# hooman007/ProtoASNet

Measured on AMD Instinct MI355X. Metric: clips/sec forward, higher is better.
Workload: dtype bf16; 1 GPU; Video ProtoASNet forward, x3d_s trunk + prototype layer (P=30, D=256, K=3), 32x16x224x224 echo clips per GPU; global_batch=32, parallelism=dp1 (independent clips, no collective), launch=hipGraph replay of the forward's launch list (one graph launch per step)

## Files before the change

protoasnet_amd/csrc/stem_mfma.hip:

```cpp
#include "common.h"
#include "igemm_epilogue.h"

namespace pasn {

constexpr int SM_ROWS = 4, SM_COLS = 56, SM_PC = 116, SM_PR = 2 * (SM_ROWS - 1) + 3, SM_RING = 6;
static_assert(SM_PC % 4 == 0 && SM_PC >= 2 * SM_COLS + 4, "whole 4-column staging units, every window inside the patch");
constexpr int SM_PF = 3;

template <typename TIN>
struct SmRaw;
template <>
struct SmRaw<float> {
    f32x4 v;
    __device__ void load(const float* p) { v = *reinterpret_cast<const f32x4*>(p); }
    __device__ float get(int e) const { return v[e]; }
};
template <>
struct SmRaw<__bf16> {
    bf16x4 v;
    __device__ void load(const __bf16* p) { v = *reinterpret_cast<const bf16x4*>(p); }
    __device__ float get(int e) const { return (float)v[e]; }
};
template <>
struct SmRaw<unsigned char> {
    unsigned v;
    __device__ void load(const unsigned char* p) { v = *reinterpret_cast<const unsigned*>(p); }
    __device__ float get(int e) const { return (float)((v >> (8 * e)) & 0xffu); }
};

template <typename TIN, int CIN>
__global__ __launch_bounds__(256, 2) void x3d_stem_mfma_kernel(const TIN* __restrict__ x, const __bf16* __restrict__ wq,
                                                               const float* __restrict__ scale, const float* __restrict__ bias,
                                                               __bf16* __restrict__ y, pasn_conv_desc d, float in_a, float in_b) {
    constexpr int NT = 1, MT = 2, BN = 32, OROW = BN + 8;
    constexpr int RPF = CIN * 3;
    constexpr int KROWS = 5 * RPF;
    constexpr int KS = (KROWS + 3) / 4;
    constexpr int SLOT = CIN * SM_PR * SM_PC;
    constexpr int UNITS = SLOT / 4;
    constexpr int UPT = (UNITS + 255) / 256;
    extern __shared__ __attribute__((aligned(16))) char smem[];
    __bf16* const ring = reinterpret_cast<__bf16*>(smem);
    __bf16* const imgs = reinterpret_cast<__bf16*>(smem + SM_RING * SLOT * 2);
    float* const scb = reinterpret_cast<float*>(smem + SM_RING * SLOT * 2 + 4 * 32 * OROW * 2);
    const int tid = threadIdx.x, lane = tid & 63, wave = __builtin_amdgcn_readfirstlane(tid >> 6);
    const int c = lane & 31, h = lane >> 5;
    const int T = d.Ti;

    const int ncol = (d.Wo + SM_COLS - 1) / SM_COLS, nrow = (d.Ho + SM_ROWS - 1) / SM_ROWS;
    int b = blockIdx.x;
    const int ct = b % ncol;
    b /= ncol;
    const int rt = b % nrow;
    const int n = b / nrow;
    const int oh0 = rt * SM_ROWS, ow0 = ct * SM_COLS;
    const int hi_base = oh0 * 2 - 1, wi_base = ow0 * 2 - 4;

    bf16x8 wa[KS];
#pragma unroll
    for (int s = 0; s < KS; ++s) wa[s] = *reinterpret_cast<const bf16x8*>(wq + ((size_t)(2 * s + h) * BN + c) * 8);
    igemm_stage_scale_bias<BN>(scb, scale, bias, 0, d.Cout_p, tid);

    const long plane = (long)d.Hi * d.Wi;
    int uoff[UPT];
    int uci[UPT];
#pragma unroll
    for (int k = 0; k < UPT; ++k) {
        const int u = tid + 256 * k;
        const int pc4 = u % (SM_PC / 4), r = (u / (SM_PC / 4)) % SM_PR, ci = u / ((SM_PC / 4) * SM_PR);
        const int hi = hi_base + r, wi = wi_base + pc4 * 4;
        const bool ok = u < UNITS && (unsigned)hi < (unsigned)d.Hi && (unsigned)wi < (unsigned)d.Wi;
        uoff[k] = ok ? hi * d.Wi + wi : -1;
        uci[k] = ci < CIN ? ci : CIN - 1;
    }
    SmRaw<TIN> raw[UPT];
    auto fetch = [&](int ti) {
#pragma unroll
        for (int k = 0; k < UPT; ++k)
            raw[k].load(x + (((long)n * CIN + uci[k]) * T + ti) * plane + (uoff[k] >= 0 ? uoff[k] : 0));
    };
    auto stage = [&](int slot, bool inside) {
        __bf16* dst = ring + slot * SLOT;
#pragma unroll
        for (int k = 0; k < UPT; ++k) {
            const int u = tid + 256 * k;
            float v[4];
#pragma unroll
            for (int e = 0; e < 4; ++e) v[e] = (inside && uoff[k] >= 0) ? fmaf(raw[k].get(e), in_a, in_b) : 0.0f;
            if (u < UNITS) store4(dst + u * 4, v);
        }
    };

    const int lane_off = (2 * wave) * SM_PC + 2 * c + 2;
    const int oh = oh0 + wave;
    const int cgs = d.Cout_p / 8;
    __bf16* const img = imgs + (size_t)wave * 32 * OROW;

    auto emit = [&](int to, const int (&sb)[5]) {
        f32x16 acc[NT][MT];
#pragma unroll
        for (int j = 0; j < MT; ++j)
#pragma unroll
            for (int r = 0; r < 16; ++r) acc[0][j][r] = 0.0f;
#pragma unroll
        for (int s = 0; s < KS; ++s) {
            auto rowoff = [&](int R) {
                const int Rc = R < KROWS ? R : KROWS - 1;
                return sb[Rc / RPF] + (((Rc % RPF) / 3) * SM_PR + (Rc % RPF) % 3) * SM_PC;
            };
            const int oa = h ? rowoff(4 * s + 2) : rowoff(4 * s + 0);
            const int ob = h ? rowoff(4 * s + 3) : rowoff(4 * s + 1);
            const __bf16* srca = ring + lane_off + oa;
            const __bf16* srcb = ring + lane_off + ob;
            bf16x8 bfr[MT];
#pragma unroll
            for (int j = 0; j < MT; ++j) {
                typedef unsigned u32x4 __attribute__((ext_vector_type(4)));
                const unsigned* pa = reinterpret_cast<const unsigned*>(srca + 64 * j);
                const unsigned* pb = reinterpret_cast<const unsigned*>(srcb + 64 * j);
                u32x4 v;
                v.x = pa[0];
                v.y = pa[1];
                v.z = pb[0];
                v.w = pb[1];
                bfr[j] = __builtin_bit_cast(bf16x8, v);
            }
#pragma unroll
            for (int j = 0; j < MT; ++j) mma32(acc[0][j], wa[s], bfr[j]);
        }
        __builtin_amdgcn_sched_group_barrier(0x100, 2 * MT * SM_PF, 0);
#pragma unroll
        for (int s = 0; s < KS; ++s) {
            __builtin_amdgcn_sched_group_barrier(0x008, MT, 0);
            if (s + SM_PF < KS) __builtin_amdgcn_sched_group_barrier(0x100, 2 * MT, 0);
        }
        igemm_epilogue<NT, MT>(acc, img, scb, nullptr, y, 0, cgs, d, lane, [&](int j, long& mbase, int& nvalid) {
            mbase = (((long)n * d.To + to) * d.Ho + oh) * d.Wo + ow0 + 32 * j;
            nvalid = oh < d.Ho ? min(min(32, SM_COLS - 32 * j), d.Wo - (ow0 + 32 * j)) : 0;
        });
    };

    const int nf = T + 4;
    int r = 0;
#pragma unroll 1
    for (int f = 0; f < nf; ++f) {
        const int ti = f - 2;
        stage(r, ti >= 0 && ti < T);
        if (ti + 1 >= 0 && ti + 1 < T) fetch(ti + 1);
        __syncthreads();
        const int to = f - 4;
        if (to >= 0) {
            int sb[5];
#pragma unroll
            for (int kt = 0; kt < 5; ++kt) {
                int q = r + 2 + kt;
                q = q >= SM_RING ? q - SM_RING : q;
                q = q >= SM_RING ? q - SM_RING : q;
                sb[kt] = q * SLOT;
            }
            emit(to, sb);
        }
        r = r + 1 == SM_RING ? 0 : r + 1;
    }
}

int x3d_stem_mfma_supported(const pasn_conv_desc& d, int out_dtype) {
    if (const char* e = tune("PASN_NO_STEM_MFMA"))
        if (e[0] == '1') return 0;
    if (out_dtype != PASN_BF16 || (d.Cin != 1 && d.Cin != 3) || d.Cout_p > 32) return 0;
    if (d.kt != 1 || d.kh != 3 || d.kw != 3 || d.st != 1 || d.sh != 2 || d.sw != 2 || d.pt != 0 || d.ph != 1 || d.pw != 1) return 0;
    if (d.Wi % 4 != 0 || d.To != d.Ti) return 0;
    if ((long)d.N * d.Cin * d.Ti * d.Hi * d.Wi >= (1L << 31)) return 0;
    return 1;
}

template <typename TIN>
static int launch_stem_mfma_t(const void* x, const void* wq, const float* scale, const float* bias, void* y, const pasn_conv_desc& d,
                              float in_a, float in_b, hipStream_t s) {
    const size_t slot = (size_t)d.Cin * SM_PR * SM_PC * 2;
    const size_t lds = SM_RING * slot + (size_t)4 * 32 * (32 + 8) * 2 + 32 * 8;
    const dim3 grid((unsigned)((long)d.N * ceil_div(d.Ho, SM_ROWS) * ceil_div(d.Wo, SM_COLS))), block(256);
    if (d.Cin == 3) {
        PASN_MAX_LDS(96 * 1024, x3d_stem_mfma_kernel<TIN, 3>);
        hipLaunchKernelGGL((x3d_stem_mfma_kernel<TIN, 3>), grid, block, lds, s, (const TIN*)x, (const __bf16*)wq, scale, bias, (__bf16*)y, d,
                           in_a, in_b);
    } else {
        hipLaunchKernelGGL((x3d_stem_mfma_kernel<TIN, 1>), grid, block, lds, s, (const TIN*)x, (const __bf16*)wq, scale, bias, (__bf16*)y, d,
                           in_a, in_b);
    }
    return check_launch("x3d_stem_mfma_kernel");
}

int launch_x3d_stem_mfma(const void* x, const void* wq, const float* scale, const float* bias, void* y, const pasn_conv_desc& d, int in_dtype,
                         float in_a, float in_b, hipStream_t s) {
    if (in_dtype == PASN_F32) return launch_stem_mfma_t<float>(x, wq, scale, bias, y, d, in_a, in_b, s);
    if (in_dtype == PASN_BF16) return launch_stem_mfma_t<__bf16>(x, wq, scale, bias, y, d, in_a, in_b, s);
    if (in_dtype == PASN_U8) return launch_stem_mfma_t<unsigned char>(x, wq, scale, bias, y, d, in_a, in_b, s);
    set_error("x3d_stem_mfma: unknown input dtype");
    return PASN_ERR_ARG;
}

}
```

protoasnet_amd/csrc/tuning.hip:

```cpp
#include "tuning.h"

#include <stdlib.h>
#include <string.h>

#include <map>
#include <mutex>
#include <string>

#include "common.h"

extern char** environ;

namespace pasn {

struct TuneEntry {
    const char* name;
    const char* cls;
    const char* doc;
};

static const TuneEntry kRegistry[] = {
    {"PASN_DWMFMA",           "route", "0: depthwise 3x3x3 stride-1 stencil on the VALU kernels instead of the matrix-core kernel (dwmfma.hip)"},
    {"PASN_DWMFMA_MAXW",      "route", "matrix-core stencil only on planes at most this wide"},
    {"PASN_DW_STATS_MFMA",    "route", "0: training forward takes the stencil's batch statistics on the VALU kernel"},
    {"PASN_DW_DGRAD_REDUCE",  "route", "0: depthwise dgrad without the fused backward sums of the producer unit"},
    {"PASN_DWWG_FUSED",       "route", "1: depthwise weight gradient with the three kt taps in one launch"},
    {"PASN_EXPDW",            "route", "0: no fused expand-conv + stencil launch (x3d_expdw.hip)"},
    {"PASN_DW_TEMPORAL",      "route", "0: depthwise (kt,1,1) convs on the generic strip kernel instead of the T-marching kernel (dwtemporal.hip)"},
    {"PASN_DW_TZ",            "route", "0: the stride-1 stencils of planes 9 .. 14 wide on dwconv3d_mfma_kernel instead of the Toeplitz kernel (dw_tz.hip); 1: the Toeplitz kernel also where its blocks do not fit one round (more than 512)"},
    {"PASN_EXPDW_TZ",         "route", "0: stride-1 fused expand + stencil launches on the block-diagonal kernel (x3d_expdw.hip) instead of the Toeplitz kernel (x3d_expdw_tz.hip)"},
    {"PASN_EXPDW_S1",         "route", "stride-1 use of the fused expand + stencil launch: 0 off, 1 the SE blocks of wide planes only"},
    {"PASN_EXPDW_FUSE",       "route", "0: fused expand + stencil step as two scheduling regions (expand, then stencil)"},
    {"PASN_EXPDW_FOLD",       "route", "0: norm_a's scale applied in the fused launch's epilogue instead of folded into the expand weights (host side, plan.py)"},
    {"PASN_HEAD_CHAIN",       "route", "0: head B as seven launches instead of the chained launch (head_chain.hip)"},
    {"PASN_NO_DGRAD_S2",      "route", "stride-2 depthwise dgrad through the generic kernel"},
    {"PASN_NO_DWMARCH",       "route", "no T-marching VALU stencil (dwmarch.hip)"},
    {"PASN_NO_DWWG_MARCH",    "route", "depthwise weight gradient without the T-marching kernel"},
    {"PASN_NO_DWWG_STRIP",    "route", "depthwise weight gradient without the strip kernel"},
    {"PASN_NO_DW_STATS",      "route", "training forward: stencil and batch statistics as two calls"},
    {"PASN_NO_FC_MFMA",       "route", "7x7 stems on the VALU kernel instead of first_conv_mfma.hip"},
    {"PASN_NO_FIRST_IM2COL",  "route", "first-layer weight gradient without the im2col path"},
    {"PASN_NO_GEMM",          "route", "no LDS-tiled GEMM for pointwise convs (gemm_pw.hip)"},
    {"PASN_NO_GEMM_BN64",     "route", "no 64-column instance of the LDS-tiled GEMM"},
    {"PASN_TCONV",            "route", "0: temporal (3,1,1) convs on the implicit-GEMM kernels instead of the weight-stationary T-marching kernel (tconv_ws.hip)"},
    {"PASN_NO_HALO",          "route", "no halo-tile implicit GEMM (igemm_halo.hip)"},
    {"PASN_NO_IGEMM",         "route", "no direct-to-LDS implicit GEMM (igemm.hip)"},
    {"PASN_NO_PACK",          "route", "1: training weights packed by torch ops instead of the one-launch pack kernel (host side, train.py)"},
    {"PASN_WGT_WIDE",         "geom",  "0: the wide pointwise weight gradient with one 32 x 32 tile per wave everywhere (no 1 x 2 / 2 x 1 tiles per wave along the wide side)"},
    {"PASN_WGT_XCD",          "geom",  "0: the wide pointwise weight gradient's tile groups as blockIdx.y (a sweep apart) instead of back to back on one XCD"},
    {"PASN_DWWG_MARCH2",      "route", "0: depthwise weight gradient by round 2's marching kernel instead of round 4's (dw_wgrad.hip)"},
    {"PASN_DWWG_CH",          "geom",  "channels per thread of the depthwise weight-gradient march (4 default, 2)"},
    {"PASN_DWWG_WT",          "geom",  "outputs per strip of the depthwise weight-gradient march at stride 1 (2 default, 3)"},
    {"PASN_DWWG_BLOCKS",      "geom",  "cap on the blocks (= partial rows) of the depthwise weight-gradient march (default 512)"},
    {"PASN_TRAIN_BLOCKS",     "geom",  "blocks an elementwise training pass is cut into (default 1024; the partial-sum workspaces scale with it)"},
    {"PASN_TRAIN_ROWS_CONTIG", "geom", "1: the elementwise training passes map Cp / 8 lanes to a row (contiguous spans, fewer idle lanes) instead of the next power of two"},
    {"PASN_NO_TRAIN_PAIR",    "route", "1: the loss recipe's two trunk passes of a training step as two passes instead of one paired pass with two statistics groups (host side, trainer.py)"},
    {"PASN_TRAIN_STREAMS",    "route", "1: weight-gradient launches of the training step on the main stream instead of a second one (host side, train.py)"},
    {"PASN_TRAIN_SIDE_DEPTH", "geom",  "side-stream weight-gradient launches outstanding before the main stream waits (default 2)"},
    {"PASN_NO_EDP",           "route", "1: no whole-block launch for the 7 x 7 stage (x3d_edp.hip)"},
    {"PASN_NO_PE",            "route", "1: no streamed project + expand pair launch for the 432-channel stage (x3d_pe.hip)"},
    {"PASN_NO_PWCONV",        "route", "no register-resident persistent pointwise conv (pwconv.hip)"},
    {"PASN_NO_PWTINY",        "route", "no one-wave-per-tile pointwise conv for small maps (pwconv_tiny.hip)"},
    {"PASN_NO_SE_ANALYTIC",   "route", "training: squeeze-excite backward without the analytic pooled-gradient path (host side, train.py)"},
    {"PASN_NO_SE_FUSE",       "route", "squeeze-excite gate never inside the stencil launch"},
    {"PASN_NO_SE_PROLOGUE",   "route", "squeeze-excite gate never in the project conv's prologue"},
    {"PASN_NO_SHORTFUSE",     "route", "strided shortcut conv as its own launch"},
    {"PASN_NO_STEM",          "route", "X3D stem as two launches"},
    {"PASN_NO_STEM_MFMA",     "route", "X3D stem on the VALU kernel instead of stem_mfma.hip"},
    {"PASN_NO_TAIL_MFMA",     "route", "training head tail without the matrix-core pooling"},
    {"PASN_NO_WGRAD_GATHER",  "route", "windowed weight gradient without the gather kernel"},
    {"PASN_NO_WGRAD_HALO",    "route", "windowed weight gradient without the halo kernel (wgrad_halo.hip)"},
    {"PASN_NO_WGRAD_LDS",     "route", "pointwise weight gradient without the LDS kernel"},
    {"PASN_NO_WGRAD_TILE",    "route", "windowed weight gradient without the tiled kernel"},
    {"PASN_NO_XPAIR",         "route", "project conv never chained with the next expand conv (pwconv_xpair.hip)"},
    {"PASN_NO_XTILE",         "route", "no X-stationary pointwise conv (pwconv_xtile.hip)"},
    {"PASN_POOL_VALU",        "route", "1: head-B pooling on the VALU kernel"},
    {"PASN_SE_FUSE_MAXC",     "route", "largest channel count whose squeeze-excite gate rides in the stencil launch (default 128)"},
    {"PASN_WGRAD_DET",        "route", "1: windowed weight gradient through fixed-order partial buffers only"},
    {"PASN_WS",               "route", "0: no weight-stationary pointwise conv (pwconv_ws.hip); 'all': every covered layer"},
    {"PASN_WSPAIR",           "route", "0: no chained pairs in the weight-stationary kernel"},
    {"PASN_WS_GATED",         "route", "0: gated (SE / Swish input) layers not on the weight-stationary kernel"},
    {"PASN_XPAIR_ALL",        "route", "1: chain every covered project / expand pair, also the narrow stage-3 ones"},
    {"PASN_XTILE_GATED",      "route", "0: gated layers not on the X-stationary kernel"},
    {"PASN_DWMFMA_TC",        "geom",  "matrix-core stencil: forced T chunk"},
    {"PASN_DWMFMA_UPB",       "geom",  "matrix-core stencil: forced units per block"},
    {"PASN_DWM_TC",           "geom",  "VALU marching stencil: forced T chunk"},
    {"PASN_DWM_WT",           "geom",  "VALU marching stencil: forced outputs per strip"},
    {"PASN_EXPDW_TC",         "geom",  "fused expand + stencil: forced T chunk"},
    {"PASN_EXPDW_UPB",        "geom",  "fused expand + stencil: forced units per block"},
    {"PASN_WS_BPC",           "geom",  "weight-stationary conv: forced blocks per channel group"},
    {"PASN_WS_MT",            "geom",  "weight-stationary conv: forced 32-row sub-tiles per wave"},
    {"PASN_WS_NS",            "geom",  "weight-stationary conv: forced stage count"},
    {"PASN_WS_PT",            "geom",  "weight-stationary conv: forced waves along positions"},
    {"PASN_WS_MINK",          "geom",  "weight-stationary conv: smallest padded K it takes (default 48)"},
    {"PASN_PE_MT",            "geom",  "streamed project + expand pair: 32-row tiles per unit (2 or 4, default 4)"},
    {"PASN_DWMFMA_ABL",       "dev",   "matrix-core stencil timing ablations (bit mask)"},
    {"PASN_EXPDW_ABL",        "dev",   "fused expand + stencil timing ablations (bit mask)"},
    {"PASN_HALO_ABL",         "dev",   "halo implicit GEMM timing ablations"},
    {"PASN_PW_ABL",           "dev",   "persistent pointwise conv timing ablations (bit mask)"},
    {"PASN_WS_ABL",           "dev",   "weight-stationary conv timing ablations (needs -DPASN_WS_ABLATE too)"},
    {"PASN_EDP_STAMPS",       "dev",   "whole-block launch of the 7 x 7 stage: in-kernel phase stamps (tools/edp_bench.py)"},
    {"PASN_TZ_STAMPS",        "dev",   "Toeplitz expand + stencil launch: in-kernel phase stamps (tools/tz_bench.py)"},
    {"PASN_PE_STAMPS",        "dev",   "streamed project + expand pair: in-kernel phase stamps (tools/pe_bench.py)"},
    {"PASN_DW_WT",            "dev",   "strip stencil: outputs per thread (4, 7, 8)"},
    {"PASN_HALO_SP",          "dev",   "halo implicit GEMM: slice pipeline on / off"},
    {"PASN_IGEMM_NT",         "dev",   "implicit GEMM: forced channel tiles per block"},
    {"PASN_IGEMM_RR",         "dev",   "implicit GEMM: round-robin tile order"},
    {"PASN_WGT_BLOCKS",       "dev",   "tiled weight gradient: target block count"},
    {"PASN_WG_TPW",           "dev",   "tiled weight gradient: tiles per wave cap"},
    {"PASN_WS_HELP",          "dev",   "weight-stationary conv: 0 = no helper waves for the input transform"},
    {"PASN_WS_ROWS",          "dev",   "weight-stationary conv: minimum rows per block"},
    {"PASN_XT_MINK",          "dev",   "X-stationary conv: smallest padded K it takes"},
};

struct Snapshot {
    std::map<std::string, std::string> set;
    std::string unknown;
};

static std::mutex g_mu;
static Snapshot* g_snap = nullptr;

static bool host_side_name(const char* n) {
    static const char* const kHost[] = {"PASN_LIB_PATH", "PASN_EXTRA_HIPCC_FLAGS", "PASN_NATIVE_RCCL", "PASN_BENCH_BACKEND", "PASN_PARITY_LOG", "PASN_TB_TORCHPROF", "PASN_KB_ACT", "PASN_HC_ABL"};
    for (const char* h : kHost)
        if (!strcmp(h, n)) return true;
    return false;
}

static Snapshot* take_snapshot() {
    Snapshot* s = new Snapshot;
    for (char** e = environ; e && *e; ++e) {
        if (strncmp(*e, "PASN_", 5)) continue;
        const char* eq = strchr(*e, '=');
        if (!eq) continue;
        const std::string name(*e, eq - *e);
        bool known = false;
        for (const TuneEntry& t : kRegistry)
            if (name == t.name) {
                known = true;
#ifndef PASN_TUNING
                if (!strcmp(t.cls, "dev")) break;
#endif
                s->set[name] = eq + 1;
                break;
            }
        if (!known && !host_side_name(name.c_str())) s->unknown += (s->unknown.empty() ? "" : " ") + name;
    }
    return s;
}

static Snapshot* snapshot() {
    std::lock_guard<std::mutex> lk(g_mu);
    if (!g_snap) g_snap = take_snapshot();
    return g_snap;
}

const char* tune(const char* name) {
    Snapshot* s = snapshot();
    if (s->set.empty()) return nullptr;
    const auto it = s->set.find(name);
    return it == s->set.end() ? nullptr : it->second.c_str();
}

}

using namespace pasn;

extern "C" void pasn_tuning_reload(void) {
    Snapshot* s = take_snapshot();
    std::lock_guard<std::mutex> lk(g_mu);
    g_snap = s;
}

extern "C" const char* pasn_tuning_get(const char* name) { return name ? tune(name) : nullptr; }

extern "C" int pasn_tuning_report(char* buf, int cap, int with_registry) {
    Snapshot* s = snapshot();
    std::string out;
    for (const auto& kv : s->set) out += kv.first + "=" + kv.second + "\n";
    if (!s->unknown.empty()) out += "unknown: " + s->unknown + "\n";
    if (with_registry)
        for (const TuneEntry& t : kRegistry) out += std::string(t.name) + "\t" + t.cls + "\t" + t.doc + "\n";
    if (buf && cap > 0) {
        const int n = (int)out.size() < cap - 1 ? (int)out.size() : cap - 1;
        memcpy(buf, out.data(), n);
        buf[n] = 0;
    }
    return (int)out.size();
}
```

Before: 12750 clips/s.

## Restructure X3D stem frame pipeline with prologue lead fetch and stage-after-MFMA

Reworks the stem's temporal loop. A prologue fetches and stages the first three frames up front, and the steady-state loop then runs the MFMA K-loop before staging the next frame into the ring, so global loads and LDS stores overlap the matrix work instead of preceding it. Per-unit offsets become advancing pointers plus an in-bounds bitmask, which cuts address arithmetic. Also adds dev-only ablation flags, compiled out unless PASN_TUNING is defined, at the cost of more registers held by the lead buffers in the prologue.

```diff
diff --git a/protoasnet_amd/csrc/stem_mfma.hip b/protoasnet_amd/csrc/stem_mfma.hip
--- a/protoasnet_amd/csrc/stem_mfma.hip
+++ b/protoasnet_amd/csrc/stem_mfma.hip
@@ -6,6 +6,15 @@
 constexpr int SM_ROWS = 4, SM_COLS = 56, SM_PC = 116, SM_PR = 2 * (SM_ROWS - 1) + 3, SM_RING = 6;
 static_assert(SM_PC % 4 == 0 && SM_PC >= 2 * SM_COLS + 4, "whole 4-column staging units, every window inside the patch");
 constexpr int SM_PF = 3;
+constexpr int SM_LEAD = 3;
+
+#ifdef PASN_TUNING
+#define PASN_STEM_ABL_PARAM , int abl
+#define PASN_STEM_ABL_VALUE , stem_abl
+#else
+#define PASN_STEM_ABL_PARAM
+#define PASN_STEM_ABL_VALUE
+#endif
 
 template <typename TIN>
 struct SmRaw;
@@ -31,7 +40,10 @@
 template <typename TIN, int CIN>
 __global__ __launch_bounds__(256, 2) void x3d_stem_mfma_kernel(const TIN* __restrict__ x, const __bf16* __restrict__ wq,
                                                                const float* __restrict__ scale, const float* __restrict__ bias,
-                                                               __bf16* __restrict__ y, pasn_conv_desc d, float in_a, float in_b) {
+                                                               __bf16* __restrict__ y, pasn_conv_desc d, float in_a, float in_b PASN_STEM_ABL_PARAM) {
+#ifndef PASN_TUNING
+    constexpr int abl = 0;
+#endif
     constexpr int NT = 1, MT = 2, BN = 32, OROW = BN + 8;
     constexpr int RPF = CIN * 3;
     constexpr int KROWS = 5 * RPF;
@@ -62,31 +74,32 @@
     igemm_stage_scale_bias<BN>(scb, scale, bias, 0, d.Cout_p, tid);
 
     const long plane = (long)d.Hi * d.Wi;
-    int uoff[UPT];
-    int uci[UPT];
+    const TIN* up[UPT];
+    unsigned uin = 0;
 #pragma unroll
     for (int k = 0; k < UPT; ++k) {
         const int u = tid + 256 * k;
         const int pc4 = u % (SM_PC / 4), r = (u / (SM_PC / 4)) % SM_PR, ci = u / ((SM_PC / 4) * SM_PR);
         const int hi = hi_base + r, wi = wi_base + pc4 * 4;
         const bool ok = u < UNITS && (unsigned)hi < (unsigned)d.Hi && (unsigned)wi < (unsigned)d.Wi;
-        uoff[k] = ok ? hi * d.Wi + wi : -1;
-        uci[k] = ci < CIN ? ci : CIN - 1;
-    }
-    SmRaw<TIN> raw[UPT];
-    auto fetch = [&](int ti) {
-#pragma unroll
-        for (int k = 0; k < UPT; ++k)
-            raw[k].load(x + (((long)n * CIN + uci[k]) * T + ti) * plane + (uoff[k] >= 0 ? uoff[k] : 0));
+        uin |= ok ? 1u << k : 0u;
+        up[k] = x + ((long)n * CIN + (ci < CIN ? ci : CIN - 1)) * T * plane + (ok ? hi * d.Wi + wi : 0);
+    }
+    auto fetch = [&](SmRaw<TIN>(&raw)[UPT], long step) {
+#pragma unroll
+        for (int k = 0; k < UPT; ++k) {
+            raw[k].load(up[k]);
+            up[k] += step;
+        }
     };
-    auto stage = [&](int slot, bool inside) {
+    auto stage = [&](int slot, const SmRaw<TIN>(&raw)[UPT], bool inside) {
         __bf16* dst = ring + slot * SLOT;
 #pragma unroll
         for (int k = 0; k < UPT; ++k) {
             const int u = tid + 256 * k;
             float v[4];
 #pragma unroll
-            for (int e = 0; e < 4; ++e) v[e] = (inside && uoff[k] >= 0) ? fmaf(raw[k].get(e), in_a, in_b) : 0.0f;
+            for (int e = 0; e < 4; ++e) v[e] = (inside && (uin >> k & 1u)) ? fmaf(raw[k].get(e), in_a, in_b) : 0.0f;
             if (u < UNITS) store4(dst + u * 4, v);
         }
     };
@@ -96,8 +109,7 @@
     const int cgs = d.Cout_p / 8;
     __bf16* const img = imgs + (size_t)wave * 32 * OROW;
 
-    auto emit = [&](int to, const int (&sb)[5]) {
-        f32x16 acc[NT][MT];
+    auto kloop = [&](f32x16(&acc)[NT][MT], const int(&sb)[5]) {
 #pragma unroll
         for (int j = 0; j < MT; ++j)
 #pragma unroll
@@ -134,32 +146,44 @@
             __builtin_amdgcn_sched_group_barrier(0x008, MT, 0);
             if (s + SM_PF < KS) __builtin_amdgcn_sched_group_barrier(0x100, 2 * MT, 0);
         }
+        __builtin_amdgcn_sched_barrier(0);
+    };
+
+    SmRaw<TIN> raw[UPT];
+    {
+        SmRaw<TIN> lead[SM_LEAD][UPT];
+#pragma unroll
+        for (int i = 0; i < SM_LEAD; ++i) fetch(lead[i], i + 1 < T ? plane : 0);
+#pragma unroll
+        for (int s = 0; s < KS; ++s) asm volatile("" ::"v"(wa[s]));
+        stage(0, lead[0], false);
+        stage(1, lead[0], false);
+#pragma unroll
+        for (int i = 0; i < SM_LEAD; ++i) stage(2 + i, lead[i], i < T);
+    }
+    if (SM_LEAD < T && !(abl & 2)) fetch(raw, plane);
+
+    int r = SM_RING - 1;
+#pragma unroll 1
+    for (int to = 0; to < T; ++to) {
+        __syncthreads();
+        int sb[5];
+#pragma unroll
+        for (int kt = 0; kt < 5; ++kt) {
+            int q = r + 1 + kt;
+            q = q >= SM_RING ? q - SM_RING : q;
+            sb[kt] = q * SLOT;
+        }
+        f32x16 acc[NT][MT];
+        kloop(acc, sb);
+        const int ti = to + SM_LEAD;
+        stage(r, raw, ti < T);
         igemm_epilogue<NT, MT>(acc, img, scb, nullptr, y, 0, cgs, d, lane, [&](int j, long& mbase, int& nvalid) {
             mbase = (((long)n * d.To + to) * d.Ho + oh) * d.Wo + ow0 + 32 * j;
             nvalid = oh < d.Ho ? min(min(32, SM_COLS - 32 * j), d.Wo - (ow0 + 32 * j)) : 0;
+            if (abl & 1) nvalid = 0;
         });
-    };
-
-    const int nf = T + 4;
-    int r = 0;
-#pragma unroll 1
-    for (int f = 0; f < nf; ++f) {
-        const int ti = f - 2;
-        stage(r, ti >= 0 && ti < T);
-        if (ti + 1 >= 0 && ti + 1 < T) fetch(ti + 1);
-        __syncthreads();
-        const int to = f - 4;
-        if (to >= 0) {
-            int sb[5];
-#pragma unroll
-            for (int kt = 0; kt < 5; ++kt) {
-                int q = r + 2 + kt;
-                q = q >= SM_RING ? q - SM_RING : q;
-                q = q >= SM_RING ? q - SM_RING : q;
-                sb[kt] = q * SLOT;
-            }
-            emit(to, sb);
-        }
+        if (ti + 1 < T && !(abl & 2)) fetch(raw, plane);
         r = r + 1 == SM_RING ? 0 : r + 1;
     }
 }
@@ -180,13 +204,16 @@
     const size_t slot = (size_t)d.Cin * SM_PR * SM_PC * 2;
     const size_t lds = SM_RING * slot + (size_t)4 * 32 * (32 + 8) * 2 + 32 * 8;
     const dim3 grid((unsigned)((long)d.N * ceil_div(d.Ho, SM_ROWS) * ceil_div(d.Wo, SM_COLS))), block(256);
+#ifdef PASN_TUNING
+    const int stem_abl = tune_dev("PASN_STEM_ABL") ? atoi(tune_dev("PASN_STEM_ABL")) : 0;
+#endif
     if (d.Cin == 3) {
         PASN_MAX_LDS(96 * 1024, x3d_stem_mfma_kernel<TIN, 3>);
         hipLaunchKernelGGL((x3d_stem_mfma_kernel<TIN, 3>), grid, block, lds, s, (const TIN*)x, (const __bf16*)wq, scale, bias, (__bf16*)y, d,
-                           in_a, in_b);
+                           in_a, in_b PASN_STEM_ABL_VALUE);
     } else {
         hipLaunchKernelGGL((x3d_stem_mfma_kernel<TIN, 1>), grid, block, lds, s, (const TIN*)x, (const __bf16*)wq, scale, bias, (__bf16*)y, d,
-                           in_a, in_b);
+                           in_a, in_b PASN_STEM_ABL_VALUE);
     }
     return check_launch("x3d_stem_mfma_kernel");
 }
diff --git a/protoasnet_amd/csrc/tuning.hip b/protoasnet_amd/csrc/tuning.hip
--- a/protoasnet_amd/csrc/tuning.hip
+++ b/protoasnet_amd/csrc/tuning.hip
@@ -99,6 +99,7 @@
     {"PASN_HALO_ABL",         "dev",   "halo implicit GEMM timing ablations"},
     {"PASN_PW_ABL",           "dev",   "persistent pointwise conv timing ablations (bit mask)"},
     {"PASN_WS_ABL",           "dev",   "weight-stationary conv timing ablations (needs -DPASN_WS_ABLATE too)"},
+    {"PASN_STEM_ABL",         "dev",   "matrix-core X3D stem timing ablations (bit mask: 1 no output stores, 2 no frame loads inside the loop)"},
     {"PASN_EDP_STAMPS",       "dev",   "whole-block launch of the 7 x 7 stage: in-kernel phase stamps (tools/edp_bench.py)"},
     {"PASN_TZ_STAMPS",        "dev",   "Toeplitz expand + stencil launch: in-kernel phase stamps (tools/tz_bench.py)"},
     {"PASN_PE_STAMPS",        "dev",   "streamed project + expand pair: in-kernel phase stamps (tools/pe_bench.py)"},
```

Result: no change. 12830 clips/s, median of 6 (+0.6%).
